# 011235813/discrete_mean_field_game

Hardware: AMD Instinct MI355X
Metric: env-steps/sec for batched d-bin population rollouts (higher is better)
Workload: dtype f32 (f64 accumulate); 1 GPU; actor_critic.train(update_every="rollout") of the drop-in class (mfg_ac2.train call surface; device-side start draw every episode, one update per 15-step rollout): d=21 topics, T=15, global batch 65536 = 65536 trajectories per GPU x 1; d=21, T=15, batch_per_gpu=65536, global_batch=65536, rng=philox4x32-10, parallelism=trajectory-sharded x1, 1 all-reduce/update

## Files before the change

discrete_mean_field_game_amd/csrc/mfg_core.h:

```cpp
#pragma once
#include <hip/hip_runtime.h>
#include <stdint.h>

#include <atomic>
#include <type_traits>

#include "../../include/mfg_hip.h"
#include "mfg_device.h"

namespace mfg {

constexpr int BLOCK = 256;
constexpr int WAVES = BLOCK / WAVE;

struct CoreArgs {
  const float* pi0;
  const int32_t* start_idx;
  int64_t num_start;
  int start_draw;
  const float* pi_alpha;
  union {
    const float* P_in;
    float* pi_start_out;
  };
  const float* pi_next_in;
  const float* reward_in;
  const double* theta;
  const double* w;
  double shift, alpha_scale, gamma;
  int64_t B;
  int d, T, reward_kind, discount_pow;
  uint64_t seed;
  uint32_t first_step;
  int step_nrows;
  uint64_t traj_offset;
  float* pi_traj;
  float* pi_next_out;
  float* reward_out;
  double* delta;
  double* g;
  float* P_out;
  const float4* htab;
  unsigned* status;
  union {
    double* part_rows;
    double* step_G;
  };
  union {
    const double* pend_G;
    const double* step_rows;
  };
  double pend_lr_c, pend_lr_a;
  double* w_out;
  double* theta_out;
  double* pend_reward_acc;
#ifdef MFG_TIMING
  unsigned long long* dbg;
#endif
};
#ifdef MFG_TIMING
#define MFG_STAMP(k) if (a.dbg && blockIdx.x == 0 && threadIdx.x == 0 && s < 4) a.dbg[s * 16 + (k)] = __builtin_amdgcn_s_memtime();
#define MFG_STAMP0(k) if (a.dbg && blockIdx.x == 0 && threadIdx.x == 0) a.dbg[(k)] = __builtin_amdgcn_s_memtime();
#define MFG_STAMPB(k) if (a.dbg && threadIdx.x == 0) a.dbg[64 + 2 * blockIdx.x + (k)] = __builtin_amdgcn_s_memtime();
#else
#define MFG_STAMP(k)
#define MFG_STAMP0(k)
#define MFG_STAMPB(k)
#endif

__host__ __device__ constexpr int core_step_red_blocks(int FO) { return (FO + WAVES - 1) / WAVES; }

__device__ __forceinline__ void reduce_rows_apply_body(const double* __restrict__ rows, int nrows, int64_t FO, double* __restrict__ G,
                                                       double lr_c, double lr_a, double count, double* __restrict__ w,
                                                       const double* theta_in, double* theta_out, double* __restrict__ reward_acc,
                                                       double* slots) {
  const int lane = threadIdx.x & (WAVE - 1), wv = threadIdx.x / WAVE;
  const int64_t k = (int64_t)blockIdx.x * WAVES + wv, F = FO - 3;
  if (k >= FO) return;
  double old_val = 0.0;
  if (lane == 0) {
    if (k < F) old_val = w[k];
    else if (k == F) old_val = *theta_in;
    else if (k == F + 1 && reward_acc) old_val = *reward_acc;
  }
  const double gk = rows_column_sum(rows, nrows, FO, k, lane);
  if (lane == 0) {
    const double inv = 1.0 / count;
    G[k] = gk;
    if (k < F) w[k] = updated_param(old_val, lr_c, gk, inv);
    else if (k == F) {
      *theta_out = updated_param(old_val, lr_a, gk, inv);
// ... 852 lines not shown
          if (k < d) r0 += redq[k];
        }
        double r = r0 + r1;
        if (!LEAN && a.reward_kind == MFG_REWARD_SYNTHETIC) r *= -0.5;
        if constexpr (LADDR) rew_t[out_o + (uint32_t)s] = (float)r;
        else
        if (LEAN || a.reward_out) a.reward_out[b * T + s] = (float)r;
        if (want_v) {
          if (par) {
            v0 = totq[2];
            v1 = totq[3];
          } else {
            int k = 0;
#pragma unroll
            for (; k + 1 < d; k += 2) {
              v0 += redq[2 * d + k];
              v1 += redq[2 * d + k + 1];
            }
            if (k < d) v0 += redq[2 * d + k];
          }
          const double v_next = (v0 + v1) + wl[Q + d];
          if (SAMPLE && s == 0) {
            double u0 = 0.0, u1 = 0.0;
            if (par) {
              u0 = totq[6];
              u1 = totq[7];
            } else {
              int kk = 0;
#pragma unroll
              for (; kk + 1 < d; kk += 2) {
                u0 += redq[3 * d + kk];
                u1 += redq[3 * d + kk + 1];
              }
              if (kk < d) u0 += redq[3 * d + kk];
            }
            v_cur = (u0 + u1) + wl[Q + d];
          }
          const double gd = (!LEAN && a.discount_pow) ? discount : a.gamma;
          const double del = r + gd * v_next - v_cur;
          if constexpr (LADDR) del_t[out_o + (uint32_t)s] = del;
          else
          if (LEAN || a.delta) a.delta[b * T + s] = del;
          if (SUMS) {
            scal[tlc * 3] = del;
            scal[tlc * 3 + 2] = (double)(float)r;
          }
          v_cur = v_next;
          discount *= a.gamma;
        }
      }
#ifdef MFG_ABL_TSUM
      if (false) {
#else
      if (TD && valid && i == gl && (LEAN || a.g)) {
#endif
        double g0 = 0.0, g1 = 0.0;
        if (par) {
          g0 = totq[4];
          g1 = totq[5];
        } else {
          int k = 0;
#pragma unroll
          for (; k + 1 < d; k += 2) {
            g0 += redq[d + k];
            g1 += redq[d + k + 1];
          }
          if (k < d) g0 += redq[d + k];
        }
        if constexpr (LADDR) g_t[out_o + (uint32_t)s] = g0 + g1;
        else
        a.g[b * T + s] = g0 + g1;
        if (SUMS) scal[tlc * 3 + 1] = g0 + g1;
      }
      if constexpr (LADDR) {
        if (valid) trj_t[trj_o + (uint32_t)((s + 1) * d)] = pi_n;
      } else
      if (valid && (LEAN || a.pi_traj)) a.pi_traj[(b * (int64_t)(T + 1) + s + 1) * d + i] = pi_n;
      pi_i = pi_n;
      MFG_STAMP(5)
    }
    if (valid && a.pi_next_out) a.pi_next_out[b * d + i] = pi_i;
    if constexpr (SUMS && SAMPLE && TD && D > 0) {
      if (a.part_rows) {
        constexpr int FO = D * (D + 1) / 2 + D + 1 + 3;
        static_assert(WAVES * FO * 8 <= WAVES * (WAVE / D) * D * (D | 1) * 4, "the partial rows reuse the tile region");
        tile_sync();
        const int li = lane & 15, lk = lane >> 4;
        const int trj = wv * G + lk;
        const bool ok = lk < G && trj < nb;
        const int trc = ok ? trj : 0;
        const bool plo_ok = li < D, phi_ok = 16 + li < D;
        const float plo = pis[trc * D + (plo_ok ? li : 0)], phi = pis[trc * D + (phi_ok ? 16 + li : 0)];
        const double de = ok ? scal[trc * 3] : 0.0, dg = ok ? scal[trc * 3 + 1] : 0.0, rr = ok ? scal[trc * 3 + 2] : 0.0;
        const double one = ok ? 1.0 : 0.0;
        auto aug = [&](int idx, float pv, bool is_pi, double& A, double& B) {
          const float ad = idx == D ? 1.0f : 0.0f, b1 = (idx == D || idx == D + 3) ? 1.0f : 0.0f;
          const double a1 = idx == D + 1 ? 1.0 : 0.0, bg = idx == D + 1 ? 1.0 : 0.0, br = idx == D + 2 ? 1.0 : 0.0;
          A = fma(de, (double)(is_pi ? pv : ad), a1 * one);
          B = fma(bg, dg, fma(br, rr, (double)(is_pi ? pv : b1)));
        };
        double A_lo, B_lo, A_hi, B_hi;
        aug(li, plo, plo_ok, A_lo, B_lo);
        aug(16 + li, phi, phi_ok, A_hi, B_hi);
        const v4d_t z = (v4d_t)(0.0);
        const v4d_t c0 = __builtin_amdgcn_mfma_f64_16x16x4f64(A_lo, B_lo, z, 0, 0, 0);
        const v4d_t c1 = __builtin_amdgcn_mfma_f64_16x16x4f64(A_lo, B_hi, z, 0, 0, 0);
        const v4d_t c2 = __builtin_amdgcn_mfma_f64_16x16x4f64(A_hi, B_hi, z, 0, 0, 0);
        __syncthreads();
        double* rows = reinterpret_cast<double*>(tile);
        constexpr int Qc = D * (D + 1) / 2, Fc = Qc + D + 1;
#pragma unroll
        for (int tt = 0; tt < 3; ++tt) {
#pragma unroll
          for (int v = 0; v < 4; ++v) {
            const int gi = (tt == 2 ? 16 : 0) + 4 * v + lk, gj = (tt == 0 ? 0 : 16) + li;
            int k = -1;
            if (gj < D) {
              if (gi <= gj) k = feat_idx(gi, gj, D);
            } else if (gj == D) {
              if (gi <= D) k = Qc + gi;
            } else if (gj == D + 1) {
              if (gi == D) k = Fc;
            } else if (gj == D + 2) {
              if (gi == D + 1) k = Fc + 1;
            } else if (gj == D + 3) {
              if (gi == D + 1) k = Fc + 2;
            }
            const double val = tt == 0 ? c0[v] : (tt == 1 ? c1[v] : c2[v]);
            if (k >= 0) rows[wv * FO + k] = val;
          }
        }
        __syncthreads();
        for (int k = tid; k < FO; k += BLOCK) {
          double tsum = rows[k];
#pragma unroll
          for (int q = 1; q < WAVES; ++q) tsum += rows[q * FO + k];
          a.part_rows[tileid * FO + k] = tsum;
        }
        __syncthreads();
      }
    }
    MFG_STAMP0(11)
    MFG_STAMPB(1)
  }
}
template <bool SAMPLE, bool TD, bool FAST, int D, bool SUMS = false, int STEP = 0>
__global__ __launch_bounds__(BLOCK, SUMS ? 2 : (FAST ? MFG_CORE_SMALL_WAVES : MFG_CORE_SMALL_WAVES_F64)) void k_core_small(CoreArgs a) { core_small_body<SAMPLE, TD, FAST, D, SUMS, STEP>(a); }
template <int D>
__global__ __launch_bounds__(BLOCK, MFG_CORE_SMALL_WAVES) void k_core_small_lean(CoreArgs a) { core_small_body<true, true, true, D, false, 0, true>(a); }
inline bool core_lean_ok(const CoreArgs& a) {
  return a.step_nrows == 0 && !a.part_rows && !a.P_out && !a.reward_in && a.reward_kind == MFG_REWARD_MFG_AC2 && !a.pi_alpha &&
         !a.pi_next_in && !a.discount_pow && a.pi_traj && a.reward_out && a.delta && a.g && a.w &&
         (!MFG_LEAN_ADDR || a.T < (1 << 20));
}

inline size_t core_small_lds(int d, bool want_v, bool sample) {
  const int G = WAVE / d, TB = WAVES * G, dp = d | 1;
  const size_t F = (size_t)d * (d + 1) / 2 + d + 1;
  const size_t fl = (size_t)TB * d * dp + 5 * (size_t)TB * d;
  return (want_v ? ((F + 1) & ~(size_t)1) * 8 : 0) + (sample ? (size_t)2 * TB * d * 8 : 0) + (size_t)4 * TB * d * 8 + (fl + (fl & 1)) * 4 +
         (size_t)TB * 3 * 8 + (size_t)TB * 8 * 8 + (size_t)TB * 2 * d * 4;
}

#ifndef MFG_CORE_LARGE_WAVES
#define MFG_CORE_LARGE_WAVES(R) (((R) <= 2 || (R) == 4) ? 3 : 2)
#endif
#ifndef MFG_CORE_LARGE_WAVES_MIXED_SAMPLING
#define MFG_CORE_LARGE_WAVES_MIXED_SAMPLING(R) ((R) <= 2 ? 4 : ((R) <= 7 ? 3 : 2))
#endif
__host__ __device__ constexpr int large_row_batch(int R, bool td) { return R <= 2 ? 8 : (R <= 4 ? (td ? 8 : 4) : 2); }
inline size_t core_large_lds(int d, bool sample, bool fast, bool td) {
  const int R = (d + WAVE - 1) / WAVE;
  if (sample && fast) return (size_t)WAVES * ((td ? 5 : 2) * d + large_row_batch(R, td) * WAVE * R) * 4;
  return (size_t)WAVES * 4 * d * 4 + (size_t)WAVES * 3 * d * 8;
}
template <int R>
__device__ __forceinline__ void stash_store(float* p, const float* y) {
  if constexpr (R % 4 == 0) {
#pragma unroll
    for (int m = 0; m < R; m += 4) *reinterpret_cast<float4*>(p + m) = make_float4(y[m], y[m + 1], y[m + 2], y[m + 3]);
  } else if constexpr (R % 2 == 0) {
#pragma unroll
    for (int m = 0; m < R; m += 2) *reinterpret_cast<float2*>(p + m) = make_float2(y[m], y[m + 1]);
  } else {
#pragma unroll
    for (int m = 0; m < R; ++m) p[m] = y[m];
  }
}
template <int R>
__device__ __forceinline__ void stash_load(float* y, const float* p) {
  if constexpr (R % 4 == 0) {
#pragma unroll
    for (int m = 0; m < R; m += 4) {
      const float4 v = *reinterpret_cast<const float4*>(p + m);
      y[m] = v.x, y[m + 1] = v.y, y[m + 2] = v.z, y[m + 3] = v.w;
    }
  } else if constexpr (R % 2 == 0) {
#pragma unroll
    for (int m = 0; m < R; m += 2) {
      const float2 v = *reinterpret_cast<const float2*>(p + m);
      y[m] = v.x, y[m + 1] = v.y;
    }
  } else {
#pragma unroll
    for (int m = 0; m < R; ++m) y[m] = p[m];
  }
}
template <int R, bool SAMPLE, bool TD, bool FAST, bool FULL>
__global__ __launch_bounds__(BLOCK, (SAMPLE && FAST) ? MFG_CORE_LARGE_WAVES_MIXED_SAMPLING(R) : MFG_CORE_LARGE_WAVES(R))
void k_core_large(CoreArgs a) {
  extern __shared__ __attribute__((aligned(16))) float smem[];
// ... 467 lines not shown
```

discrete_mean_field_game_amd/csrc/mfg_grad.h:

```cpp
#pragma once
#include <hip/hip_runtime.h>
#include <stdint.h>

#include "mfg_core.h"

using namespace mfg;

constexpr int MFG_GRAD_SMALL_MAX_D = 28;
constexpr int GR_OUT_PER_THREAD = 4;
constexpr int GR_OUT_PER_BLOCK = GR_OUT_PER_THREAD * BLOCK;

struct GradArgs {
  const float* pi;
  int64_t stride_b;
  const double* delta;
  const double* g;
  const float* reward;
  int64_t N;
  int T, d, chunk;
  int64_t nsb;
  double* partial;
  int add_reward;
  unsigned* counter;
  double* G;
  int accumulate, apply;
  double lr_c, lr_a;
  double *w, *theta, *reward_acc;
};

__device__ __forceinline__ void grad_partial_body(const GradArgs& a) {
  extern __shared__ __attribute__((aligned(16))) unsigned char smem_raw[];
  const int d = a.d, Q = d * (d + 1) / 2, F = Q + d + 1, FO = F + 3;
  double* dl = reinterpret_cast<double*>(smem_raw);
  float* sp = reinterpret_cast<float*>(dl + 3 * a.chunk);
  const int tid = threadIdx.x;
  int oi[GR_OUT_PER_THREAD], oj[GR_OUT_PER_THREAD], kind[GR_OUT_PER_THREAD];
  double acc[GR_OUT_PER_THREAD];
#pragma unroll
  for (int u = 0; u < GR_OUT_PER_THREAD; ++u) {
    const int k = blockIdx.y * GR_OUT_PER_BLOCK + u * BLOCK + tid;
    acc[u] = 0.0;
    oi[u] = oj[u] = 0;
    if (k < Q) {
      int i = (int)(((2.0 * d + 1.0) - sqrt((2.0 * d + 1.0) * (2.0 * d + 1.0) - 8.0 * (double)k)) * 0.5);
      while (i > 0 && feat_idx(i, i, d) > k) --i;
      while (i + 1 < d && feat_idx(i + 1, i + 1, d) <= k) ++i;
      oi[u] = i;
      oj[u] = i + (k - feat_idx(i, i, d));
      kind[u] = 0;
    } else if (k < Q + d) {
      oi[u] = k - Q;
      kind[u] = 1;
    } else if (k < FO) {
      kind[u] = 2 + (k - (Q + d));
    } else {
      kind[u] = -1;
    }
  }
  for (int64_t n0 = (int64_t)blockIdx.x * a.chunk; n0 < a.N; n0 += a.nsb * a.chunk) {
    const int cn = (int)((a.N - n0) < a.chunk ? (a.N - n0) : a.chunk);
    __syncthreads();
    for (int k = tid; k < cn * d; k += BLOCK) {
      const int q = k / d, c = k - q * d;
      const int64_t n = n0 + q;
      const int64_t b = n / a.T;
      const int s = (int)(n - b * a.T);
      sp[k] = a.pi[b * a.stride_b + (int64_t)s * d + c];
    }
    for (int q = tid; q < cn; q += BLOCK) {
      const double de = a.delta[n0 + q];
      dl[3 * q] = de;
      dl[3 * q + 1] = a.g ? de * a.g[n0 + q] : 0.0;
      dl[3 * q + 2] = a.reward ? (double)a.reward[n0 + q] : 0.0;
    }
    __syncthreads();
#pragma unroll
    for (int u = 0; u < GR_OUT_PER_THREAD; ++u) {
      double s_ = acc[u];
      if (kind[u] == 0) {
        for (int q = 0; q < cn; ++q) s_ = fma(dl[3 * q] * (double)sp[q * d + oi[u]], (double)sp[q * d + oj[u]], s_);
      } else if (kind[u] == 1) {
        for (int q = 0; q < cn; ++q) s_ = fma(dl[3 * q], (double)sp[q * d + oi[u]], s_);
      } else if (kind[u] == 2) {
        for (int q = 0; q < cn; ++q) s_ += dl[3 * q];
      } else if (kind[u] == 3) {
        for (int q = 0; q < cn; ++q) s_ += dl[3 * q + 1];
      } else if (kind[u] == 4) {
        for (int q = 0; q < cn; ++q) s_ += dl[3 * q + 2];
      } else if (kind[u] == 5) {
        s_ += (double)cn;
      }
      acc[u] = s_;
    }
  }
#pragma unroll
  for (int u = 0; u < GR_OUT_PER_THREAD; ++u) {
    const int k = blockIdx.y * GR_OUT_PER_BLOCK + u * BLOCK + tid;
    if (kind[u] >= 0) a.partial[(int64_t)blockIdx.x * FO + k] = acc[u];
  }
}

constexpr int GS_CH = 64;
#ifndef MFG_GS_BPC
#define MFG_GS_BPC 2
#endif

template <int D>
struct GradChunk {
  static constexpr int NL = D ? D : MFG_GRAD_SMALL_MAX_D;
  float pi[NL];
  double de, dg;
  float rr;
};

constexpr int MFG_GRAD_LONG_T = 1 << 22;
__device__ __forceinline__ int grad_boundaries_wide(int sj, int T, float invT) {
  return T >= GS_CH ? (int)(sj >= T) : (int)(((float)sj + 0.5f) * invT);
}
template <int D, bool WIDE>
__device__ __forceinline__ void grad_chunk_load(GradChunk<D>& c, const GradArgs& a, const double* gp, const float* rp, int d,
                                                int64_t n0, int64_t b0, int s0, int lane, float invT, float inv_d) {
  const int last = (int)((a.N - 1 - n0) < (GS_CH - 1) ? (a.N - 1 - n0) : (GS_CH - 1));
  {
    const int64_t n = n0 + (lane < last ? lane : last);
    c.de = a.delta[n];
    c.dg = gp[n];
    c.rr = rp[n];
  }
  if constexpr (!WIDE) {
    const float* cb = a.pi + b0 * a.stride_b + (int64_t)s0 * d;
    const int extra = (int)(a.stride_b - (int64_t)a.T * d);
#pragma unroll
    for (int k = 0; k < GradChunk<D>::NL; ++k) {
      if (!D && k * WAVE >= GS_CH * d) {
        c.pi[k] = 0.0f;
        continue;
      }
      int e = k * WAVE + lane;
      int j = (int)(((float)e + 0.5f) * inv_d);
      if (j > last) { j = last; e = last * d; }
      const int q = (int)(((float)(s0 + j) + 0.5f) * invT);
      c.pi[k] = cb[(unsigned)(e + __mul24(q, extra))];
    }
  } else {
#pragma unroll
    for (int k = 0; k < GradChunk<D>::NL; ++k) {
      if (!D && k * WAVE >= GS_CH * d) {
        c.pi[k] = 0.0f;
        continue;
      }
      const int e = k * WAVE + lane;
      int j = (int)(((float)e + 0.5f) * inv_d);
      int col = e - j * d;
      if (j > last) { j = last; col = 0; }
      const int sj = s0 + j;
      const int q = grad_boundaries_wide(sj, a.T, invT);
      const int64_t off = (b0 + q) * a.stride_b + ((int64_t)(sj - q * a.T) * d + col);
      c.pi[k] = a.pi[off];
    }
  }
}

template <int D, bool WIDE>
__device__ __forceinline__ void grad_mfma_small_body(const GradArgs& a) {
  const int d = D ? D : a.d;
  const int Q = d * (d + 1) / 2, F = Q + d + 1, FO = F + 3;
  constexpr int DMAX = D ? D : MFG_GRAD_SMALL_MAX_D;
  constexpr int PI_FL = GS_CH * DMAX + 16;
  constexpr int W_BYTES = ((PI_FL * 4 + 15) / 16) * 16 + GS_CH * 3 * 8;
  constexpr int RED_BYTES = WAVES * 3 * 4 * WAVE * 8;
  __shared__ __attribute__((aligned(16))) unsigned char smem[(WAVES * W_BYTES > RED_BYTES) ? WAVES * W_BYTES : RED_BYTES];
  const int tid = threadIdx.x, lane = tid & (WAVE - 1), wv = __builtin_amdgcn_readfirstlane(tid / WAVE);
  float* lpi = reinterpret_cast<float*>(smem + (size_t)wv * W_BYTES);
  double* lsc = reinterpret_cast<double*>(smem + (size_t)wv * W_BYTES + ((PI_FL * 4 + 15) / 16) * 16);
  const int li = lane & 15, lk = lane >> 4;
  auto consts = [&](int idx, float& a_d, double& a_1, float& b_1, double& b_g, double& b_r) {
    a_d = idx == d ? 1.0f : 0.0f;
    a_1 = idx == d + 1 ? 1.0 : 0.0;
    b_1 = (idx == d || idx == d + 3) ? 1.0f : 0.0f;
    b_g = idx == d + 1 ? 1.0 : 0.0;
    b_r = idx == d + 2 ? 1.0 : 0.0;
  };
  float ad_lo, b1_lo, ad_hi, b1_hi;
  double a1_lo, a1_hi, bg_lo, br_lo, bg_hi, br_hi;
  consts(li, ad_lo, a1_lo, b1_lo, bg_lo, br_lo);
  consts(16 + li, ad_hi, a1_hi, b1_hi, bg_hi, br_hi);
  const bool pi_lo = li < d, pi_hi = 16 + li < d;
  const int ilo = pi_lo ? li : 0, ihi = pi_hi ? 16 + li : 0;
  const bool has_g = a.g != nullptr, has_r = a.reward != nullptr;
  const double* gp = has_g ? a.g : a.delta;
  const float* rp = has_r ? a.reward : a.pi;
  v4d_t c00 = (v4d_t)(0.0), c01 = (v4d_t)(0.0), c11 = (v4d_t)(0.0);
  const float invT = 1.0f / (float)a.T, inv_d = 1.0f / (float)d;
  const int64_t NC = (a.N + GS_CH - 1) / GS_CH;
  const int64_t W = (int64_t)gridDim.x * WAVES;
  const int64_t gw = (int64_t)blockIdx.x * WAVES + wv;
  GradChunk<D> nx;
  if (gw < NC) grad_chunk_load<D, WIDE>(nx, a, gp, rp, d, gw * GS_CH, (gw * GS_CH) / a.T, (int)((gw * GS_CH) % a.T), lane, invT, inv_d);
  for (int64_t ch = gw; ch < NC; ch += W) {
    const int64_t n0 = ch * GS_CH;
    __builtin_amdgcn_s_waitcnt(0xc07f);
    __builtin_amdgcn_wave_barrier();
#pragma unroll
    for (int k = 0; k < GradChunk<D>::NL; ++k)
      if (D || k * WAVE < GS_CH * d) lpi[k * WAVE + lane] = nx.pi[k];
    {
      const bool ok = n0 + lane < a.N;
      const double rr = (ok && has_r) ? (double)nx.rr : 0.0;
      double de = ok ? nx.de : 0.0;
      if (a.add_reward) {
        de += rr;
        if (ok) const_cast<double*>(a.delta)[n0 + lane] = de;
      }
      lsc[3 * lane] = de;
      lsc[3 * lane + 1] = (ok && has_g) ? nx.dg : 0.0;
      lsc[3 * lane + 2] = rr;
    }
    const int nvalid = (int)((a.N - n0) < GS_CH ? (a.N - n0) : GS_CH);
    if (ch + W < NC) {
      const int64_t n1 = (ch + W) * GS_CH;
      grad_chunk_load<D, WIDE>(nx, a, gp, rp, d, n1, n1 / a.T, (int)(n1 % a.T), lane, invT, inv_d);
    }
    __builtin_amdgcn_s_waitcnt(0xc07f);
    __builtin_amdgcn_wave_barrier();
#pragma unroll 4
    for (int ks = 0; ks < GS_CH / 4; ++ks) {
      const int j = 4 * ks + lk;
      const float plo = lpi[j * d + ilo], phi = lpi[j * d + ihi];
      const double de = lsc[3 * j], dg = lsc[3 * j + 1];
      const double rr = lsc[3 * j + 2];
      const double one = j < nvalid ? 1.0 : 0.0;
      double A_lo, B_lo;
      if constexpr (D >= 16) {
        B_lo = (double)plo;
        A_lo = de * B_lo;
      } else {
        A_lo = fma(de, (double)(pi_lo ? plo : ad_lo), a1_lo * one);
        B_lo = fma(bg_lo, dg, fma(br_lo, rr, (double)(pi_lo ? plo : b1_lo)));
      }
      const double A_hi = fma(de, (double)(pi_hi ? phi : ad_hi), a1_hi * one);
      const double B_hi = fma(bg_hi, dg, fma(br_hi, rr, (double)(pi_hi ? phi : b1_hi)));
      c00 = __builtin_amdgcn_mfma_f64_16x16x4f64(A_lo, B_lo, c00, 0, 0, 0);
      c01 = __builtin_amdgcn_mfma_f64_16x16x4f64(A_lo, B_hi, c01, 0, 0, 0);
      c11 = __builtin_amdgcn_mfma_f64_16x16x4f64(A_hi, B_hi, c11, 0, 0, 0);
    }
  }
  __syncthreads();
  double (*red)[3][4][WAVE] = reinterpret_cast<double (*)[3][4][WAVE]>(smem);
#pragma unroll
  for (int v = 0; v < 4; ++v) {
    red[wv][0][v][lane] = c00[v];
    red[wv][1][v][lane] = c01[v];
    red[wv][2][v][lane] = c11[v];
  }
  __syncthreads();
  double* out = a.partial + (int64_t)blockIdx.x * FO;
  for (int e = tid; e < 3 * 4 * WAVE; e += BLOCK) {
    const int t = e / (4 * WAVE), v = (e / WAVE) & 3, l = e & (WAVE - 1);
    const int gi = (t == 2 ? 16 : 0) + 4 * v + (l >> 4), gj = (t == 0 ? 0 : 16) + (l & 15);
    int k = -1;
    if (gj < d) {
      if (gi <= gj) k = feat_idx(gi, gj, d);
    } else if (gj == d) {
      if (gi <= d) k = Q + gi;
    } else if (gj == d + 1) {
      if (gi == d) k = F;
    } else if (gj == d + 2) {
      if (gi == d + 1) k = F + 1;
    } else if (gj == d + 3) {
      if (gi == d + 1) k = F + 2;
    }
    if (k >= 0) {
      double tsum = red[0][t][v][l];
#pragma unroll
      for (int q = 1; q < WAVES; ++q) tsum += red[q][t][v][l];
      out[k] = tsum;
    }
  }
  if (!a.counter) return;
  __shared__ int s_last;
  __threadfence();
  __syncthreads();
  if (tid == 0) s_last = (atomicAdd(a.counter, 1u) == gridDim.x - 1) ? 1 : 0;
  __syncthreads();
  if (!s_last) return;
  __threadfence();
  double* fin = &red[0][0][0][0];
  const int nrows = (int)gridDim.x;
  for (int k = tid; k < FO; k += BLOCK) {
    double s0 = 0.0, s1 = 0.0, s2 = 0.0, s3 = 0.0;
    const double* col = a.partial + k;
    int r = 0;
    for (; r + 7 < nrows; r += 8) {
      const double v0 = col[(int64_t)r * FO], v1 = col[(int64_t)(r + 1) * FO], v2 = col[(int64_t)(r + 2) * FO],
                   v3 = col[(int64_t)(r + 3) * FO], v4 = col[(int64_t)(r + 4) * FO], v5 = col[(int64_t)(r + 5) * FO],
                   v6 = col[(int64_t)(r + 6) * FO], v7 = col[(int64_t)(r + 7) * FO];
      s0 += v0;
      s1 += v1;
      s2 += v2;
      s3 += v3;
      s0 += v4;
      s1 += v5;
      s2 += v6;
      s3 += v7;
    }
    for (; r < nrows; ++r) s0 += col[(int64_t)r * FO];
    const double tot = (s0 + s1) + (s2 + s3);
    const double gk = a.accumulate ? a.G[k] + tot : tot;
    a.G[k] = gk;
    fin[k] = gk;
  }
  __syncthreads();
  if (a.apply) {
    const double count = fin[F + 2];
    if (count > 0.0) {
      const double inv = 1.0 / count;
      for (int k = tid; k < F; k += BLOCK) a.w[k] = updated_param(a.w[k], a.lr_c, fin[k], inv);
      if (tid == 0) {
        if (a.reward_acc) *a.reward_acc += fin[F + 1] * inv;
        *a.theta = updated_param(*a.theta, a.lr_a, fin[F], inv);
      }
    }
  }
  if (tid == 0) *a.counter = 0u;
}
template <int D, bool WIDE = false>
__global__ __launch_bounds__(BLOCK) void k_grad_mfma_small(GradArgs a) { grad_mfma_small_body<D, WIDE>(a); }

constexpr int GM_KC = 32;
#ifndef MFG_GM_TPW
#define MFG_GM_TPW 8
#endif
constexpr int GM_TPW = MFG_GM_TPW;

template <int NPF>
__device__ __forceinline__ void grad_mfma_body(const GradArgs& a, int tpw) {
  extern __shared__ __attribute__((aligned(16))) unsigned char smem_raw[];
  const int d = a.d, nt = d >> 4, pitch = d + 16;
  const int Q = d * (d + 1) / 2, F = Q + d + 1, FO = F + 3;
  double* dl = reinterpret_cast<double*>(smem_raw);
  double* red = dl + GM_KC;
  float* sp = reinterpret_cast<float*>(red + 4 * BLOCK);
  const int tid = threadIdx.x, lane = tid & (WAVE - 1), wv = tid / WAVE;
  const int ntiles = nt * (nt + 1) / 2;
  const int t0 = ((int)blockIdx.y * WAVES + wv) * tpw;
  int nmine = ntiles - t0;
  nmine = nmine < 0 ? 0 : (nmine > tpw ? tpw : nmine);
  int tr[GM_TPW], tc[GM_TPW];
#pragma unroll
  for (int i = 0; i < GM_TPW; ++i) {
    int t = t0 + i, r = 0;
    if (i < nmine) {
      while (t >= nt - r) {
        t -= nt - r;
        ++r;
      }
    } else {
      t = 0;
    }
    tr[i] = r;
    tc[i] = r + t;
  }
  v4d_t acc[GM_TPW];
#pragma unroll
  for (int i = 0; i < GM_TPW; ++i) acc[i] = (v4d_t)(0.0);
  const bool side = blockIdx.y == 0;
  double lin[4] = {0.0, 0.0, 0.0, 0.0}, s_d = 0.0, s_dg = 0.0, s_r = 0.0, s_n = 0.0;
  const int li = lane & 15, lk = lane >> 4;
  const double invT = 1.0 / (double)a.T;
  const int dq = d >> 2, rpp = BLOCK / (dq > 0 ? dq : 1);
  const int q0 = tid / dq, c4 = tid - q0 * dq;
  float4 pf[NPF > 0 ? NPF : 1];
  double pf_de = 0.0, pf_dg = 0.0, pf_rr = 0.0;
  bool pf_on = false;
#define MFG_GM_FETCH(n0_)                                                                              \
  {                                                                                                    \
    const int cn_ = (int)((a.N - (n0_)) < GM_KC ? (a.N - (n0_)) : GM_KC);                              \
    _Pragma("unroll") for (int u = 0; u < NPF; ++u) {                                                  \
      const int q = q0 + u * rpp;                                                                      \
      pf[u] = make_float4(0.f, 0.f, 0.f, 0.f);                                                         \
      if (q < cn_) {                                                                                   \
        const int64_t n = (n0_) + q;                                                                   \
        const int64_t b = (int64_t)(((double)n + 0.5) * invT);                                         \
        pf[u] = *reinterpret_cast<const float4*>(a.pi + b * a.stride_b + (n - b * a.T) * d + 4 * c4);  \
      }                                                                                                \
    }                                                                                                  \
    pf_de = 0.0; pf_dg = 0.0; pf_rr = 0.0; pf_on = false;                                              \
    if (tid < cn_) {                                                                                   \
      const int64_t n = (n0_) + tid;                                                                   \
      pf_de = a.delta[n];                                                                              \
      pf_rr = a.reward ? (double)a.reward[n] : 0.0;                                                    \
      if (a.g) pf_dg = a.g[n];                                                                         \
      pf_on = true;                                                                                    \
    }                                                                                                  \
  }
  if (NPF > 0 && (int64_t)blockIdx.x * GM_KC < a.N) MFG_GM_FETCH((int64_t)blockIdx.x * GM_KC)
  for (int64_t n0 = (int64_t)blockIdx.x * GM_KC; n0 < a.N; n0 += (int64_t)gridDim.x * GM_KC) {
    const int cn = (int)((a.N - n0) < GM_KC ? (a.N - n0) : GM_KC);
    __syncthreads();
    if (NPF > 0) {
#pragma unroll
      for (int u = 0; u < NPF; ++u) *reinterpret_cast<float4*>(sp + (q0 + u * rpp) * pitch + 4 * c4) = pf[u];
      if (tid < GM_KC) {
        if (side && pf_on) {
          s_d += pf_de;
          if (a.g) s_dg = fma(pf_de, pf_dg, s_dg);
          s_r += pf_rr;
// ... 182 lines not shown
```

Baseline: 1.107 billion env-steps/s.

## Cover the batch Gram sums with two MFMA tiles instead of three for d=21

Introduces a compile-time two-tile cover that packs the upper-triangular Gram entries and augmented columns for d=21 and d=15 into two 16x16 f64 MFMA tiles, where three were used before. Both the in-rollout partial-row sums and the standalone gradient kernel now issue two MFMAs per step, with lane plans and output index tables computed by constexpr code and checked by static_asserts. The goal is to cut f64 MFMA work and reduction shared-memory traffic by about a third, at the cost of extra per-lane select logic and more complex table-driven indexing.

```diff
diff --git a/discrete_mean_field_game_amd/csrc/mfg_core.h b/discrete_mean_field_game_amd/csrc/mfg_core.h
--- a/discrete_mean_field_game_amd/csrc/mfg_core.h
+++ b/discrete_mean_field_game_amd/csrc/mfg_core.h
@@ -7,6 +7,7 @@
 
 #include "../../include/mfg_hip.h"
 #include "mfg_device.h"
+#include "mfg_grad_cover.h"
 
 namespace mfg {
 
@@ -1025,6 +1026,8 @@
     if (valid && a.pi_next_out) a.pi_next_out[b * d + i] = pi_i;
     if constexpr (SUMS && SAMPLE && TD && D > 0) {
       if (a.part_rows) {
+        static_assert(D == 21 || D == 15, "the in-kernel sums use the two-tile cover");
+        using C = GradCover<D>;
         constexpr int FO = D * (D + 1) / 2 + D + 1 + 3;
         static_assert(WAVES * FO * 8 <= WAVES * (WAVE / D) * D * (D | 1) * 4, "the partial rows reuse the tile region");
         tile_sync();
@@ -1032,44 +1035,26 @@
         const int trj = wv * G + lk;
         const bool ok = lk < G && trj < nb;
         const int trc = ok ? trj : 0;
-        const bool plo_ok = li < D, phi_ok = 16 + li < D;
-        const float plo = pis[trc * D + (plo_ok ? li : 0)], phi = pis[trc * D + (phi_ok ? 16 + li : 0)];
+        const unsigned pl = C::P.lane[li], fl = pl >> 10;
+        const float px = pis[trc * D + (int)(pl & 31u)], py = pis[trc * D + (int)(pl >> 5 & 31u)];
         const double de = ok ? scal[trc * 3] : 0.0, dg = ok ? scal[trc * 3 + 1] : 0.0, rr = ok ? scal[trc * 3 + 2] : 0.0;
         const double one = ok ? 1.0 : 0.0;
-        auto aug = [&](int idx, float pv, bool is_pi, double& A, double& B) {
-          const float ad = idx == D ? 1.0f : 0.0f, b1 = (idx == D || idx == D + 3) ? 1.0f : 0.0f;
-          const double a1 = idx == D + 1 ? 1.0 : 0.0, bg = idx == D + 1 ? 1.0 : 0.0, br = idx == D + 2 ? 1.0 : 0.0;
-          A = fma(de, (double)(is_pi ? pv : ad), a1 * one);
-          B = fma(bg, dg, fma(br, rr, (double)(is_pi ? pv : b1)));
-        };
-        double A_lo, B_lo, A_hi, B_hi;
-        aug(li, plo, plo_ok, A_lo, B_lo);
-        aug(16 + li, phi, phi_ok, A_hi, B_hi);
+        const float xs = (fl & C::X_LIVE) ? px : 1.0f, ys = (fl & C::Y_LIVE) ? py : ((fl & C::Y_ONE) ? 1.0f : 0.0f);
+        const double B_1 = (double)xs;
+        const double A_1 = de * B_1;
+        const double A_2 = fma(de, (double)((fl & C::A2_X) ? xs : ys), ((fl & C::A2_ONE) ? 1.0 : 0.0) * one);
+        const double B_2 = fma((fl & C::B2_G) ? 1.0 : 0.0, dg, fma((fl & C::B2_R) ? 1.0 : 0.0, rr, (double)((fl & C::B2_X) ? xs : ys)));
         const v4d_t z = (v4d_t)(0.0);
-        const v4d_t c0 = __builtin_amdgcn_mfma_f64_16x16x4f64(A_lo, B_lo, z, 0, 0, 0);
-        const v4d_t c1 = __builtin_amdgcn_mfma_f64_16x16x4f64(A_lo, B_hi, z, 0, 0, 0);
-        const v4d_t c2 = __builtin_amdgcn_mfma_f64_16x16x4f64(A_hi, B_hi, z, 0, 0, 0);
+        const v4d_t c0 = __builtin_amdgcn_mfma_f64_16x16x4f64(A_1, B_1, z, 0, 0, 0);
+        const v4d_t c1 = __builtin_amdgcn_mfma_f64_16x16x4f64(A_2, B_2, z, 0, 0, 0);
         __syncthreads();
         double* rows = reinterpret_cast<double*>(tile);
-        constexpr int Qc = D * (D + 1) / 2, Fc = Qc + D + 1;
-#pragma unroll
-        for (int tt = 0; tt < 3; ++tt) {
+#pragma unroll
+        for (int tt = 0; tt < 2; ++tt) {
 #pragma unroll
           for (int v = 0; v < 4; ++v) {
-            const int gi = (tt == 2 ? 16 : 0) + 4 * v + lk, gj = (tt == 0 ? 0 : 16) + li;
-            int k = -1;
-            if (gj < D) {
-              if (gi <= gj) k = feat_idx(gi, gj, D);
-            } else if (gj == D) {
-              if (gi <= D) k = Qc + gi;
-            } else if (gj == D + 1) {
-              if (gi == D) k = Fc;
-            } else if (gj == D + 2) {
-              if (gi == D + 1) k = Fc + 1;
-            } else if (gj == D + 3) {
-              if (gi == D + 1) k = Fc + 2;
-            }
-            const double val = tt == 0 ? c0[v] : (tt == 1 ? c1[v] : c2[v]);
+            const int k = C::T.k[tt][4 * v + lk][li];
+            const double val = tt == 0 ? c0[v] : c1[v];
             if (k >= 0) rows[wv * FO + k] = val;
           }
         }
diff --git a/discrete_mean_field_game_amd/csrc/mfg_grad.h b/discrete_mean_field_game_amd/csrc/mfg_grad.h
--- a/discrete_mean_field_game_amd/csrc/mfg_grad.h
+++ b/discrete_mean_field_game_amd/csrc/mfg_grad.h
@@ -3,6 +3,7 @@
 #include <stdint.h>
 
 #include "mfg_core.h"
+#include "mfg_grad_cover.h"
 
 using namespace mfg;
 
@@ -166,9 +167,11 @@
   const int d = D ? D : a.d;
   const int Q = d * (d + 1) / 2, F = Q + d + 1, FO = F + 3;
   constexpr int DMAX = D ? D : MFG_GRAD_SMALL_MAX_D;
+  constexpr bool COVER = D == 21 || D == 15;
+  constexpr int NT = COVER ? 2 : 3;
   constexpr int PI_FL = GS_CH * DMAX + 16;
   constexpr int W_BYTES = ((PI_FL * 4 + 15) / 16) * 16 + GS_CH * 3 * 8;
-  constexpr int RED_BYTES = WAVES * 3 * 4 * WAVE * 8;
+  constexpr int RED_BYTES = WAVES * NT * 4 * WAVE * 8;
   __shared__ __attribute__((aligned(16))) unsigned char smem[(WAVES * W_BYTES > RED_BYTES) ? WAVES * W_BYTES : RED_BYTES];
   const int tid = threadIdx.x, lane = tid & (WAVE - 1), wv = __builtin_amdgcn_readfirstlane(tid / WAVE);
   float* lpi = reinterpret_cast<float*>(smem + (size_t)wv * W_BYTES);
@@ -185,8 +188,24 @@
   double a1_lo, a1_hi, bg_lo, br_lo, bg_hi, br_hi;
   consts(li, ad_lo, a1_lo, b1_lo, bg_lo, br_lo);
   consts(16 + li, ad_hi, a1_hi, b1_hi, bg_hi, br_hi);
-  const bool pi_lo = li < d, pi_hi = 16 + li < d;
-  const int ilo = pi_lo ? li : 0, ihi = pi_hi ? 16 + li : 0;
+  bool pi_lo = li < d, pi_hi = 16 + li < d;
+  int ilo = pi_lo ? li : 0, ihi = pi_hi ? 16 + li : 0;
+  bool a2_x = false, b2_x = false;
+  if constexpr (COVER) {
+    using C = GradCover<D>;
+    const unsigned pl = C::P.lane[li], fl = pl >> 10;
+    ilo = (int)(pl & 31u);
+    ihi = (int)(pl >> 5 & 31u);
+    pi_lo = fl & C::X_LIVE;
+    pi_hi = fl & C::Y_LIVE;
+    b1_lo = 1.0f;
+    b1_hi = (fl & C::Y_ONE) ? 1.0f : 0.0f;
+    a2_x = fl & C::A2_X;
+    b2_x = fl & C::B2_X;
+    a1_hi = (fl & C::A2_ONE) ? 1.0 : 0.0;
+    bg_hi = (fl & C::B2_G) ? 1.0 : 0.0;
+    br_hi = (fl & C::B2_R) ? 1.0 : 0.0;
+  }
   const bool has_g = a.g != nullptr, has_r = a.reward != nullptr;
   const double* gp = has_g ? a.g : a.delta;
   const float* rp = has_r ? a.reward : a.pi;
@@ -230,6 +249,15 @@
       const double de = lsc[3 * j], dg = lsc[3 * j + 1];
       const double rr = lsc[3 * j + 2];
       const double one = j < nvalid ? 1.0 : 0.0;
+      if constexpr (COVER) {
+        const float xs = pi_lo ? plo : b1_lo, ys = pi_hi ? phi : b1_hi;
+        const double B_1 = (double)xs;
+        const double A_1 = de * B_1;
+        const double A_2 = fma(de, (double)(a2_x ? xs : ys), a1_hi * one);
+        const double B_2 = fma(bg_hi, dg, fma(br_hi, rr, (double)(b2_x ? xs : ys)));
+        c00 = __builtin_amdgcn_mfma_f64_16x16x4f64(A_1, B_1, c00, 0, 0, 0);
+        c01 = __builtin_amdgcn_mfma_f64_16x16x4f64(A_2, B_2, c01, 0, 0, 0);
+      } else {
       double A_lo, B_lo;
       if constexpr (D >= 16) {
         B_lo = (double)plo;
@@ -243,23 +271,26 @@
       c00 = __builtin_amdgcn_mfma_f64_16x16x4f64(A_lo, B_lo, c00, 0, 0, 0);
       c01 = __builtin_amdgcn_mfma_f64_16x16x4f64(A_lo, B_hi, c01, 0, 0, 0);
       c11 = __builtin_amdgcn_mfma_f64_16x16x4f64(A_hi, B_hi, c11, 0, 0, 0);
+      }
     }
   }
   __syncthreads();
-  double (*red)[3][4][WAVE] = reinterpret_cast<double (*)[3][4][WAVE]>(smem);
+  double (*red)[NT][4][WAVE] = reinterpret_cast<double (*)[NT][4][WAVE]>(smem);
 #pragma unroll
   for (int v = 0; v < 4; ++v) {
     red[wv][0][v][lane] = c00[v];
     red[wv][1][v][lane] = c01[v];
-    red[wv][2][v][lane] = c11[v];
+    if constexpr (!COVER) red[wv][2][v][lane] = c11[v];
   }
   __syncthreads();
   double* out = a.partial + (int64_t)blockIdx.x * FO;
-  for (int e = tid; e < 3 * 4 * WAVE; e += BLOCK) {
+  for (int e = tid; e < NT * 4 * WAVE; e += BLOCK) {
     const int t = e / (4 * WAVE), v = (e / WAVE) & 3, l = e & (WAVE - 1);
     const int gi = (t == 2 ? 16 : 0) + 4 * v + (l >> 4), gj = (t == 0 ? 0 : 16) + (l & 15);
     int k = -1;
-    if (gj < d) {
+    if constexpr (COVER) {
+      k = GradCover<D>::T.k[t][4 * v + (l >> 4)][l & 15];
+    } else if (gj < d) {
       if (gi <= gj) k = feat_idx(gi, gj, d);
     } else if (gj == d) {
       if (gi <= d) k = Q + gi;
diff --git a/discrete_mean_field_game_amd/csrc/mfg_grad_cover.h b/discrete_mean_field_game_amd/csrc/mfg_grad_cover.h
--- /dev/null
+++ b/discrete_mean_field_game_amd/csrc/mfg_grad_cover.h
@@ -0,0 +1,115 @@
+#pragma once
+#include <stdint.h>
+
+template <int D>
+struct GradCoverDef {
+  static_assert(D == 21 || D == 15, "two-tile cover: d = 21 and 15");
+  static constexpr int NS = D - 15, Q = D * (D + 1) / 2, F = Q + D + 1, FO = F + 3;
+  struct Tables {
+    int8_t row[2][16], col[2][16];
+    int16_t k[2][16][16];
+    int16_t pos[FO];
+    int16_t times[FO];
+  };
+  static constexpr int out_of(int ai, int bj) {
+    if (ai < 0 || bj < 0) return -1;
+    if (ai < D && bj < D) return ai <= bj ? ai * D - (ai * (ai - 1)) / 2 + (bj - ai) : -1;
+    if (ai <= D && bj == D) return Q + ai;
+    if (ai == D && bj == D + 1) return F;
+    if (ai == D + 1 && bj == D + 2) return F + 1;
+    if (ai == D + 1 && bj == D) return F + 2;
+    return -1;
+  }
+  static constexpr Tables make() {
+    Tables t{};
+    for (int l = 0; l < 16; ++l) {
+      t.row[0][l] = (int8_t)(l < 8 ? l : l < 15 ? l + NS : D);
+      t.col[0][l] = (int8_t)(l < 8 ? l : l < 15 ? l + NS : D);
+      t.row[1][l] = (int8_t)(l < 8 ? l : l < 14 ? (l - 8 < NS ? l : -1) : l == 14 ? D : D + 1);
+      t.col[1][l] = (int8_t)(l < 6 ? (l < NS ? 8 + l : -1) : l == 6 ? D : l == 7 ? D + 1 : l < 15 ? l + NS : D + 2);
+    }
+    for (int o = 0; o < FO; ++o) t.pos[o] = -1, t.times[o] = 0;
+    for (int tl = 0; tl < 2; ++tl)
+      for (int r = 0; r < 16; ++r)
+        for (int c = 0; c < 16; ++c) {
+          int o = out_of(t.row[tl][r], t.col[tl][c]);
+          if (tl == 1 && o >= 0)
+            for (int r1 = 0; r1 < 16; ++r1)
+              for (int c1 = 0; c1 < 16; ++c1)
+                if (t.k[0][r1][c1] == o) o = -1;
+          t.k[tl][r][c] = (int16_t)o;
+          if (o >= 0) {
+            t.pos[o] = (int16_t)(tl << 8 | r << 4 | c);
+            ++t.times[o];
+          }
+        }
+    return t;
+  }
+};
+template <int D>
+struct GradCover : GradCoverDef<D> {
+  using GradCoverDef<D>::FO;
+  static constexpr typename GradCoverDef<D>::Tables T = GradCoverDef<D>::make();
+  static constexpr bool state(int id) { return id >= 0 && id < D; }
+  static constexpr bool every_output_once() {
+    for (int o = 0; o < FO; ++o)
+      if (T.times[o] != 1 || T.pos[o] < 0) return false;
+    return true;
+  }
+  static constexpr bool pairs_row_le_column() {
+    for (int tl = 0; tl < 2; ++tl)
+      for (int r = 0; r < 16; ++r)
+        for (int c = 0; c < 16; ++c)
+          if (T.k[tl][r][c] >= 0 && state(T.row[tl][r]) && state(T.col[tl][c]) && T.row[tl][r] > T.col[tl][c]) return false;
+    return true;
+  }
+  static constexpr bool ids_in_range() {
+    for (int tl = 0; tl < 2; ++tl)
+      for (int l = 0; l < 16; ++l)
+        if (T.row[tl][l] < -1 || T.row[tl][l] > D + 1 || T.col[tl][l] < -1 || T.col[tl][l] > D + 2) return false;
+    return true;
+  }
+  static constexpr bool a2x(int l) { return state(T.row[1][l]) && T.row[1][l] == T.row[0][l]; }
+  static constexpr bool a2y(int l) { return state(T.row[1][l]) && !a2x(l); }
+  static constexpr bool b2x(int l) { return state(T.col[1][l]) && T.col[1][l] == T.row[0][l]; }
+  static constexpr bool b2y(int l) { return state(T.col[1][l]) && !b2x(l); }
+  static constexpr int a2c(int l) { return T.row[1][l] == D ? 1 : 0; }
+  static constexpr int b2c(int l) { return T.col[1][l] == D ? 1 : 0; }
+  static constexpr bool two_reads_per_lane() {
+    for (int l = 0; l < 16; ++l) {
+      const int r1 = T.row[0][l], c1 = T.col[0][l];
+      if (!((state(r1) && c1 == r1) || (r1 == D && c1 == D))) return false;
+      if (a2y(l) && b2y(l) && T.row[1][l] != T.col[1][l]) return false;
+      if (a2y(l) && !b2x(l) && !b2y(l)) return false;
+      if (b2y(l) && !a2x(l) && !a2y(l)) return false;
+      if (!a2x(l) && !a2y(l) && !b2x(l) && !b2y(l) && a2c(l) != b2c(l)) return false;
+    }
+    return true;
+  }
+  enum : unsigned { X_LIVE = 1, Y_LIVE = 2, Y_ONE = 4, A2_X = 8, B2_X = 16, A2_ONE = 32, B2_G = 64, B2_R = 128 };
+  struct Plans { uint32_t lane[16]; };
+  static constexpr Plans plans() {
+    Plans p{};
+    for (int l = 0; l < 16; ++l) {
+      const int xi = state(T.row[0][l]) ? T.row[0][l] : 0;
+      const int yi = a2y(l) ? T.row[1][l] : b2y(l) ? T.col[1][l] : 0;
+      const int yc = !(a2x(l) || a2y(l)) ? a2c(l) : !(b2x(l) || b2y(l)) ? b2c(l) : 0;
+      const unsigned f = (state(T.row[0][l]) ? X_LIVE : 0u) | ((a2y(l) || b2y(l)) ? Y_LIVE : 0u) | (yc ? Y_ONE : 0u) |
+                         (a2x(l) ? A2_X : 0u) | (b2x(l) ? B2_X : 0u) | (T.row[1][l] == D + 1 ? A2_ONE : 0u) |
+                         (T.col[1][l] == D + 1 ? B2_G : 0u) | (T.col[1][l] == D + 2 ? B2_R : 0u);
+      p.lane[l] = (uint32_t)xi | (uint32_t)yi << 5 | f << 10;
+    }
+    return p;
+  }
+  static constexpr Plans P = plans();
+};
+template <int D>
+constexpr bool grad_cover_proved() {
+  using C = GradCover<D>;
+  static_assert(C::ids_in_range(), "cover: unknown entry id");
+  static_assert(C::every_output_once(), "cover: an entry of G is missing or kept twice");
+  static_assert(C::pairs_row_le_column(), "cover: a kept pair has its larger index in the row");
+  static_assert(C::two_reads_per_lane(), "cover: a lane needs more than its two state reads");
+  return true;
+}
+static_assert(grad_cover_proved<21>() && grad_cover_proved<15>(), "two-tile cover of the d = 21 / 15 batch sums");
```

After: 1.116 billion env-steps/s (median of 6 runs). Within noise of the previous version (+0.8%).

## Cover augmented gradient Gram matrix with two MFMA tiles for d=21 and 15

Applied to the files above, without the earlier changes.

Adds a two-tile gradient kernel for d=21 and d=15. A compile-time map packs the upper-triangular Gram, linear, and scalar entries into two 16x16 f64 MFMA tiles instead of three, with a static_assert that every output entry is produced exactly once. The scale factors (delta, dg, reward, valid flag) are stored per row in LDS so operands come from table lookups instead of per-lane selects. This cuts one MFMA and some operand arithmetic per k-step and shrinks the reduction buffer. In exchange it adds a more complex index map and a padded LDS row layout, and it moves the shared finish code into a helper.

```diff
diff --git a/discrete_mean_field_game_amd/csrc/mfg_grad.h b/discrete_mean_field_game_amd/csrc/mfg_grad.h
--- a/discrete_mean_field_game_amd/csrc/mfg_grad.h
+++ b/discrete_mean_field_game_amd/csrc/mfg_grad.h
@@ -161,8 +161,228 @@
   }
 }
 
+__device__ __forceinline__ void grad_small_finish(const GradArgs& a, double* fin, int F, int FO, int tid) {
+  if (!a.counter) return;
+  __shared__ int s_last;
+  __threadfence();
+  __syncthreads();
+  if (tid == 0) s_last = (atomicAdd(a.counter, 1u) == gridDim.x - 1) ? 1 : 0;
+  __syncthreads();
+  if (!s_last) return;
+  __threadfence();
+  const int nrows = (int)gridDim.x;
+  for (int k = tid; k < FO; k += BLOCK) {
+    double s0 = 0.0, s1 = 0.0, s2 = 0.0, s3 = 0.0;
+    const double* col = a.partial + k;
+    int r = 0;
+    for (; r + 7 < nrows; r += 8) {
+      const double v0 = col[(int64_t)r * FO], v1 = col[(int64_t)(r + 1) * FO], v2 = col[(int64_t)(r + 2) * FO],
+                   v3 = col[(int64_t)(r + 3) * FO], v4 = col[(int64_t)(r + 4) * FO], v5 = col[(int64_t)(r + 5) * FO],
+                   v6 = col[(int64_t)(r + 6) * FO], v7 = col[(int64_t)(r + 7) * FO];
+      s0 += v0;
+      s1 += v1;
+      s2 += v2;
+      s3 += v3;
+      s0 += v4;
+      s1 += v5;
+      s2 += v6;
+      s3 += v7;
+    }
+    for (; r < nrows; ++r) s0 += col[(int64_t)r * FO];
+    const double tot = (s0 + s1) + (s2 + s3);
+    const double gk = a.accumulate ? a.G[k] + tot : tot;
+    a.G[k] = gk;
+    fin[k] = gk;
+  }
+  __syncthreads();
+  if (a.apply) {
+    const double count = fin[F + 2];
+    if (count > 0.0) {
+      const double inv = 1.0 / count;
+      for (int k = tid; k < F; k += BLOCK) a.w[k] = updated_param(a.w[k], a.lr_c, fin[k], inv);
+      if (tid == 0) {
+        if (a.reward_acc) *a.reward_acc += fin[F + 1] * inv;
+        *a.theta = updated_param(*a.theta, a.lr_a, fin[F], inv);
+      }
+    }
+  }
+  if (tid == 0) *a.counter = 0u;
+}
+
+template <int D>
+struct GradTileSets;
+template <>
+struct GradTileSets<21> {
+  static constexpr int R[2][16] = {{0, 1, 2, 3, 4, 5, 6, 7, 8, 9, 10, 11, 12, 13, 14, 15},
+                                   {0, 1, 2, 3, 4, 5, 16, 17, 18, 19, 20, 21, 22, -1, -1, -1}};
+  static constexpr int C[2][16] = {{6, 7, 8, 9, 10, 11, 12, 13, 14, 15, 16, 17, 18, 19, 20, 21},
+                                   {0, 1, 2, 3, 4, 5, 16, 17, 18, 19, 20, 21, 22, 23, 24, -1}};
+};
+template <>
+struct GradTileSets<15> {
+  static constexpr int R[2][16] = {{0, 1, 2, 3, 4, 5, 6, 7, 8, 9, 10, 11, 12, 13, 14, 15},
+                                   {15, 16, -1, -1, -1, -1, -1, -1, -1, -1, -1, -1, -1, -1, -1, -1}};
+  static constexpr int C[2][16] = {{0, 1, 2, 3, 4, 5, 6, 7, 8, 9, 10, 11, 12, 13, 14, 15},
+                                   {16, 17, 18, -1, -1, -1, -1, -1, -1, -1, -1, -1, -1, -1, -1, -1}};
+};
+template <int D>
+constexpr bool grad_two_tiles = D == 21 || D == 15;
+
+constexpr int grad_aug_out(int i, int j, int d) {
+  const int Q = d * (d + 1) / 2, F = Q + d + 1;
+  if (i < 0 || j < 0) return -1;
+  if (j < d) return i <= j ? i * d - (i * (i - 1)) / 2 + (j - i) : -1;
+  if (j == d) return i <= d ? Q + i : -1;
+  if (j == d + 1) return i == d ? F : -1;
+  if (j == d + 2) return i == d + 1 ? F + 1 : -1;
+  if (j == d + 3) return i == d + 1 ? F + 2 : -1;
+  return -1;
+}
+constexpr int GS_DE = 0, GS_DG = 1, GS_RR = 2, GS_ONE = 3, GS_SC = 4;
+template <int D>
+struct GradTileMap {
+  short out[2][16][16];
+  unsigned char a_off[2][16], a_sc[2][16], b_off[2][16], b_sc[2][16];
+  constexpr GradTileMap() : out{}, a_off{}, a_sc{}, b_off{}, b_sc{} {
+    using S = GradTileSets<D>;
+    for (int t = 0; t < 2; ++t)
+      for (int s = 0; s < 16; ++s) {
+        const int i = S::R[t][s], j = S::C[t][s];
+        a_off[t][s] = (unsigned char)(i >= 0 && i < D ? i : D);
+        a_sc[t][s] = (unsigned char)(i == D + 1 ? GS_ONE : GS_DE);
+        b_off[t][s] = (unsigned char)(j >= 0 && j < D ? j : D);
+        b_sc[t][s] = (unsigned char)(j == D + 1 ? GS_DG : j == D + 2 ? GS_RR : GS_ONE);
+        for (int c = 0; c < 16; ++c) {
+          bool in0 = false;
+          if (t == 1)
+            for (int s0 = 0; s0 < 16; ++s0)
+              for (int c0 = 0; c0 < 16; ++c0) in0 = in0 || (S::R[0][s0] == i && S::C[0][c0] == S::C[1][c]);
+          out[t][s][c] = (short)(in0 ? -1 : grad_aug_out(i, S::C[t][c], D));
+        }
+      }
+  }
+  constexpr bool valid() const {
+    constexpr int FO = D * (D + 1) / 2 + D + 4;
+    int n[FO] = {};
+    for (int t = 0; t < 2; ++t)
+      for (int s = 0; s < 16; ++s)
+        for (int c = 0; c < 16; ++c)
+          if (out[t][s][c] >= FO) return false;
+          else if (out[t][s][c] >= 0) ++n[out[t][s][c]];
+    for (int k = 0; k < FO; ++k)
+      if (n[k] != 1) return false;
+    for (int s = 0; s < 16; ++s) {
+      const int i = GradTileSets<D>::R[0][s], j = GradTileSets<D>::C[0][s];
+      if (i > D || (j > D && j != D + 3)) return false;
+    }
+    return true;
+  }
+};
+template <int D>
+struct GradTiles {
+  static constexpr GradTileMap<D> map{};
+};
+static_assert(GradTiles<21>::map.valid() && GradTiles<15>::map.valid(),
+              "the two tiles must supply every one of the F + 3 entries of G exactly once");
+
+#ifndef MFG_GS2_UNROLL
+#define MFG_GS2_UNROLL 4
+#endif
 template <int D, bool WIDE>
-__device__ __forceinline__ void grad_mfma_small_body(const GradArgs& a) {
+__device__ __forceinline__ void grad_mfma_two_tile_body(const GradArgs& a) {
+  using TT = GradTiles<D>;
+  constexpr int d = D, Q = d * (d + 1) / 2, F = Q + d + 1, FO = F + 3;
+  constexpr int RS = D + 1;
+  constexpr int PI_BYTES = GS_CH * RS * 4;
+  constexpr int W_BYTES = PI_BYTES + GS_CH * GS_SC * 8;
+  constexpr int RED_BYTES = WAVES * 2 * 4 * WAVE * 8;
+  static_assert(FO * 8 <= RED_BYTES, "the finish keeps G in the reduction's space");
+  __shared__ __attribute__((aligned(16))) unsigned char smem[(WAVES * W_BYTES > RED_BYTES) ? WAVES * W_BYTES : RED_BYTES];
+  const int tid = threadIdx.x, lane = tid & (WAVE - 1), wv = __builtin_amdgcn_readfirstlane(tid / WAVE);
+  float* lrow = reinterpret_cast<float*>(smem + (size_t)wv * W_BYTES);
+  double* lsc = reinterpret_cast<double*>(smem + (size_t)wv * W_BYTES + PI_BYTES);
+  const int li = lane & 15, lk = lane >> 4;
+  const float* rA0 = lrow + lk * RS + TT::map.a_off[0][li];
+  const float* rB0 = lrow + lk * RS + TT::map.b_off[0][li];
+  const float* rA1 = lrow + lk * RS + TT::map.a_off[1][li];
+  const float* rB1 = lrow + lk * RS + TT::map.b_off[1][li];
+  const double* sD = lsc + lk * GS_SC + GS_DE;
+  const double* sA1 = lsc + lk * GS_SC + TT::map.a_sc[1][li];
+  const double* sB1 = lsc + lk * GS_SC + TT::map.b_sc[1][li];
+  int park[D];
+#pragma unroll
+  for (int k = 0; k < D; ++k) park[k] = (k * WAVE + lane) + (k * WAVE + lane) / D;
+  lrow[lane * RS + D] = 1.0f;
+  const bool has_g = a.g != nullptr, has_r = a.reward != nullptr;
+  const double* gp = has_g ? a.g : a.delta;
+  const float* rp = has_r ? a.reward : a.pi;
+  v4d_t c0 = (v4d_t)(0.0), c1 = (v4d_t)(0.0);
+  const float invT = 1.0f / (float)a.T, inv_d = 1.0f / (float)d;
+  const int64_t NC = (a.N + GS_CH - 1) / GS_CH;
+  const int64_t W = (int64_t)gridDim.x * WAVES;
+  const int64_t gw = (int64_t)blockIdx.x * WAVES + wv;
+  GradChunk<D> nx;
+  if (gw < NC) grad_chunk_load<D, WIDE>(nx, a, gp, rp, d, gw * GS_CH, (gw * GS_CH) / a.T, (int)((gw * GS_CH) % a.T), lane, invT, inv_d);
+  for (int64_t ch = gw; ch < NC; ch += W) {
+    const int64_t n0 = ch * GS_CH;
+    __builtin_amdgcn_s_waitcnt(0xc07f);
+    __builtin_amdgcn_wave_barrier();
+#pragma unroll
+    for (int k = 0; k < D; ++k) lrow[park[k]] = nx.pi[k];
+    {
+      const bool ok = n0 + lane < a.N;
+      const double rr = (ok && has_r) ? (double)nx.rr : 0.0;
+      double de = ok ? nx.de : 0.0;
+      if (a.add_reward) {
+        de += rr;
+        if (ok) const_cast<double*>(a.delta)[n0 + lane] = de;
+      }
+      lsc[GS_SC * lane + GS_DE] = de;
+      lsc[GS_SC * lane + GS_DG] = (ok && has_g) ? nx.dg : 0.0;
+      lsc[GS_SC * lane + GS_RR] = rr;
+      lsc[GS_SC * lane + GS_ONE] = fma(de, 0.0, ok ? 1.0 : 0.0);
+    }
+    if (ch + W < NC) {
+      const int64_t n1 = (ch + W) * GS_CH;
+      grad_chunk_load<D, WIDE>(nx, a, gp, rp, d, n1, n1 / a.T, (int)(n1 % a.T), lane, invT, inv_d);
+    }
+    __builtin_amdgcn_s_waitcnt(0xc07f);
+    __builtin_amdgcn_wave_barrier();
+#pragma unroll MFG_GS2_UNROLL
+    for (int ks = 0; ks < GS_CH / 4; ++ks) {
+      const int ro = 4 * ks * RS, so = 4 * ks * GS_SC;
+      const double A0 = sD[so] * (double)rA0[ro];
+      const double B0 = (double)rB0[ro];
+      const double A1 = sA1[so] * (double)rA1[ro];
+      const double B1 = (double)rB1[ro] * sB1[so];
+      c0 = __builtin_amdgcn_mfma_f64_16x16x4f64(A0, B0, c0, 0, 0, 0);
+      c1 = __builtin_amdgcn_mfma_f64_16x16x4f64(A1, B1, c1, 0, 0, 0);
+    }
+  }
+  __syncthreads();
+  double (*red)[2][4][WAVE] = reinterpret_cast<double (*)[2][4][WAVE]>(smem);
+#pragma unroll
+  for (int v = 0; v < 4; ++v) {
+    red[wv][0][v][lane] = c0[v];
+    red[wv][1][v][lane] = c1[v];
+  }
+  __syncthreads();
+  double* out = a.partial + (int64_t)blockIdx.x * FO;
+  for (int e = tid; e < 2 * 4 * WAVE; e += BLOCK) {
+    const int t = e / (4 * WAVE), v = (e / WAVE) & 3, l = e & (WAVE - 1);
+    const int k = TT::map.out[t][4 * v + (l >> 4)][l & 15];
+    if (k >= 0) {
+      double tsum = red[0][t][v][l];
+#pragma unroll
+      for (int q = 1; q < WAVES; ++q) tsum += red[q][t][v][l];
+      out[k] = tsum;
+    }
+  }
+  grad_small_finish(a, &red[0][0][0][0], F, FO, tid);
+}
+
+template <int D, bool WIDE>
+__device__ __forceinline__ void grad_mfma_three_tile_body(const GradArgs& a) {
   const int d = D ? D : a.d;
   const int Q = d * (d + 1) / 2, F = Q + d + 1, FO = F + 3;
   constexpr int DMAX = D ? D : MFG_GRAD_SMALL_MAX_D;
@@ -230,14 +450,8 @@
       const double de = lsc[3 * j], dg = lsc[3 * j + 1];
       const double rr = lsc[3 * j + 2];
       const double one = j < nvalid ? 1.0 : 0.0;
-      double A_lo, B_lo;
-      if constexpr (D >= 16) {
-        B_lo = (double)plo;
-        A_lo = de * B_lo;
-      } else {
-        A_lo = fma(de, (double)(pi_lo ? plo : ad_lo), a1_lo * one);
-        B_lo = fma(bg_lo, dg, fma(br_lo, rr, (double)(pi_lo ? plo : b1_lo)));
-      }
+      const double A_lo = fma(de, (double)(pi_lo ? plo : ad_lo), a1_lo * one);
+      const double B_lo = fma(bg_lo, dg, fma(br_lo, rr, (double)(pi_lo ? plo : b1_lo)));
       const double A_hi = fma(de, (double)(pi_hi ? phi : ad_hi), a1_hi * one);
       const double B_hi = fma(bg_hi, dg, fma(br_hi, rr, (double)(pi_hi ? phi : b1_hi)));
       c00 = __builtin_amdgcn_mfma_f64_16x16x4f64(A_lo, B_lo, c00, 0, 0, 0);
@@ -277,52 +491,12 @@
       out[k] = tsum;
     }
   }
-  if (!a.counter) return;
-  __shared__ int s_last;
-  __threadfence();
-  __syncthreads();
-  if (tid == 0) s_last = (atomicAdd(a.counter, 1u) == gridDim.x - 1) ? 1 : 0;
-  __syncthreads();
-  if (!s_last) return;
-  __threadfence();
-  double* fin = &red[0][0][0][0];
-  const int nrows = (int)gridDim.x;
-  for (int k = tid; k < FO; k += BLOCK) {
-    double s0 = 0.0, s1 = 0.0, s2 = 0.0, s3 = 0.0;
-    const double* col = a.partial + k;
-    int r = 0;
-    for (; r + 7 < nrows; r += 8) {
-      const double v0 = col[(int64_t)r * FO], v1 = col[(int64_t)(r + 1) * FO], v2 = col[(int64_t)(r + 2) * FO],
-                   v3 = col[(int64_t)(r + 3) * FO], v4 = col[(int64_t)(r + 4) * FO], v5 = col[(int64_t)(r + 5) * FO],
-                   v6 = col[(int64_t)(r + 6) * FO], v7 = col[(int64_t)(r + 7) * FO];
-      s0 += v0;
-      s1 += v1;
-      s2 += v2;
-      s3 += v3;
-      s0 += v4;
-      s1 += v5;
-      s2 += v6;
-      s3 += v7;
-    }
-    for (; r < nrows; ++r) s0 += col[(int64_t)r * FO];
-    const double tot = (s0 + s1) + (s2 + s3);
-    const double gk = a.accumulate ? a.G[k] + tot : tot;
-    a.G[k] = gk;
-    fin[k] = gk;
-  }
-  __syncthreads();
-  if (a.apply) {
-    const double count = fin[F + 2];
-    if (count > 0.0) {
-      const double inv = 1.0 / count;
-      for (int k = tid; k < F; k += BLOCK) a.w[k] = updated_param(a.w[k], a.lr_c, fin[k], inv);
-      if (tid == 0) {
-        if (a.reward_acc) *a.reward_acc += fin[F + 1] * inv;
-        *a.theta = updated_param(*a.theta, a.lr_a, fin[F], inv);
-      }
-    }
-  }
-  if (tid == 0) *a.counter = 0u;
+  grad_small_finish(a, &red[0][0][0][0], F, FO, tid);
+}
+template <int D, bool WIDE>
+__device__ __forceinline__ void grad_mfma_small_body(const GradArgs& a) {
+  if constexpr (grad_two_tiles<D>) grad_mfma_two_tile_body<D, WIDE>(a);
+  else grad_mfma_three_tile_body<D, WIDE>(a);
 }
 template <int D, bool WIDE = false>
 __global__ __launch_bounds__(BLOCK) void k_grad_mfma_small(GradArgs a) { grad_mfma_small_body<D, WIDE>(a); }
```

Result: no change. 1.109 billion env-steps/s before, 1.118 billion env-steps/s after (median of 6 runs) (+0.8%).
